# SymbioticLab/FedScale

Measured on AMD Instinct MI355X. Metric: client-updates/sec + HBM GB/s, device-resident FedAvg reduce of KxP fp32, higher is better.
Workload: dtype f32

## Files before the change

### fedscale_amd/csrc/clip_reduce.hip

```cpp
#pragma clang fp contract(off)

#include <hip/hip_runtime.h>
#include <stdint.h>

#include "../../include/fedclip.h"
#include "fa_device.h"
#include "fa_common.h"

namespace {

struct NormGeo {
  int V, U, waves, grid_pct;
};
constexpr NormGeo NQ_NARROW{8, 4, 2, 400};
constexpr NormGeo NQ_WIDE{16, 2, 4, 75};
constexpr int64_t NQ_WIDE_MIN_P = 4LL << 20;
constexpr NormGeo norm_geo(int64_t P) { return P >= NQ_WIDE_MIN_P ? NQ_WIDE : NQ_NARROW; }

struct NormArgs {
  const f4* x;
  int64_t ld4;
  int64_t P4f;
  int64_t tiles;
  int n;
  const f4* last;
  double* ws;
};

__device__ __forceinline__ double sq_acc(double acc, f4 t, f4 l) {
  const f4 d = t - l;
  acc = __builtin_fma((double)d.x, (double)d.x, acc);
  acc = __builtin_fma((double)d.y, (double)d.y, acc);
  acc = __builtin_fma((double)d.z, (double)d.z, acc);
  acc = __builtin_fma((double)d.w, (double)d.w, acc);
  return acc;
}

template <int NQ_V, int NQ_U, int NQ_WAVES>
__global__ __launch_bounds__(64 * NQ_WAVES) void k_row_sqnorm(NormArgs r) {
  constexpr int64_t NQ_TILE4 = 64 * NQ_V;
  const int lane = threadIdx.x & 63;
  const int wave = threadIdx.x >> 6;
  const f4 z4 = f4{0.f, 0.f, 0.f, 0.f};
  for (int64_t wt = (int64_t)blockIdx.x * NQ_WAVES + wave; wt < r.tiles; wt += (int64_t)gridDim.x * NQ_WAVES) {
    const int64_t c0 = wt * NQ_TILE4 + lane;
    bool ok[NQ_V];
    f4 l[NQ_V];
#pragma unroll
    for (int j = 0; j < NQ_V; ++j) {
      ok[j] = (c0 + 64 * j) < r.P4f;
      l[j] = ok[j] ? r.last[c0 + 64 * j] : z4;
    }
    const f4* row = r.x + c0;
    double* w = r.ws + wt;
    int k = 0;
    for (; k + NQ_U <= r.n; k += NQ_U) {
      f4 t[NQ_U][NQ_V];
#pragma unroll
      for (int u = 0; u < NQ_U; ++u)
#pragma unroll
        for (int j = 0; j < NQ_V; ++j) t[u][j] = ok[j] ? __builtin_nontemporal_load(row + u * r.ld4 + 64 * j) : z4;
#pragma unroll
      for (int u = 0; u < NQ_U; ++u) {
        double acc = 0.0;
#pragma unroll
        for (int j = 0; j < NQ_V; ++j) acc = sq_acc(acc, t[u][j], l[j]);
        acc = wave_sum(acc);
        if (lane == 0) w[(int64_t)(k + u) * r.tiles] = acc;
      }
      row += NQ_U * r.ld4;
    }
    for (; k < r.n; ++k) {
      double acc = 0.0;
#pragma unroll
      for (int j = 0; j < NQ_V; ++j)
        acc = sq_acc(acc, ok[j] ? __builtin_nontemporal_load(row + 64 * j) : z4, l[j]);
      acc = wave_sum(acc);
      if (lane == 0) w[(int64_t)k * r.tiles] = acc;
      row += r.ld4;
    }
  }
}

__global__ __launch_bounds__(64) void k_sqnorm_sum(const double* __restrict__ ws, int64_t tiles,
                                                   const float* __restrict__ x, int64_t ld, int64_t P4f, int64_t P,
                                                   const float* __restrict__ last, double* __restrict__ sq) {
  const int64_t k = blockIdx.x;
  const int lane = threadIdx.x;
  double acc = 0.0;
  for (int64_t t = lane; t < tiles; t += 64) acc = acc + ws[k * tiles + t];
  acc = wave_sum(acc);
  if (lane == 0) {
    for (int64_t p = 4 * P4f; p < P; ++p) {
      const float d = x[k * ld + p] - last[p];
      acc = __builtin_fma((double)d, (double)d, acc);
    }
    sq[k] = acc;
  }
}

int64_t norm_tiles(int64_t P) {
  const int64_t tile4 = 64 * norm_geo(P).V;
  return (P / 4 + tile4 - 1) / tile4;
}
int64_t norm_grid(int64_t cus, int64_t P) {
  const NormGeo g = norm_geo(P);
  const int64_t wgs = (norm_tiles(P) + g.waves - 1) / g.waves;
  const int64_t cap = cus * g.grid_pct / 100 > 0 ? cus * g.grid_pct / 100 : 1;
  return wgs < cap ? wgs : cap;
}

__global__ __launch_bounds__(256) void k_clip_coef(const double* __restrict__ sq, int n, double M,
                                                   float* __restrict__ c, int32_t* rejected) {
  const int i = blockIdx.x * 256 + threadIdx.x;
  if (i >= n) return;
  const double s = sq[i];
  float ck = 0.0f;
  if (!__builtin_isfinite(s)) {
    atomicAdd(rejected, 1);
  } else {
    const double rk = M / (sqrt(s) + 1e-6);
    ck = rk < 1.0 ? (float)rk : 1.0f;
  }
  c[i] = ck;
}

constexpr int FCL_WAVES = 4;

struct ClipArgs {
  const f4* x;
  int64_t ld4;
  int64_t P4;
  int64_t P;
  int64_t c0;
  int64_t ntiles;
  int n;
  int flags;
  const f4* last;
  const float* coef;
  const f4* acc_in;
  float* out;
};

template <int V, int U>
__device__ __forceinline__ void clip_tile(const ClipArgs& r, int64_t tile, int lane, int wave) {
  const int64_t c0 = r.c0 + (tile * FCL_WAVES + wave) * (64LL * V) + lane;
  const f4 z4 = f4{0.f, 0.f, 0.f, 0.f};
  bool ok[V];
  f4 l[V], s[V];
#pragma unroll
  for (int j = 0; j < V; ++j) {
    ok[j] = (c0 + 64 * j) < r.P4;
    l[j] = ok[j] ? r.last[c0 + 64 * j] : z4;
    s[j] = ((r.flags & FA_ACCUMULATE) && ok[j]) ? r.acc_in[c0 + 64 * j] : z4;
  }
  const f4* row = r.x + c0;
  int k = 0;
  for (; k + U <= r.n; k += U) {
    f4 t[U][V];
#pragma unroll
    for (int u = 0; u < U; ++u)
#pragma unroll
      for (int j = 0; j < V; ++j) t[u][j] = ok[j] ? __builtin_nontemporal_load(row + u * r.ld4 + 64 * j) : z4;
#pragma unroll
    for (int u = 0; u < U; ++u) {
      const float ck = r.coef[k + u];
      if (ck != 0.0f) {
#pragma unroll
        for (int j = 0; j < V; ++j) s[j] = s[j] + ck * (t[u][j] - l[j]);
      }
    }
    row += U * r.ld4;
  }
  for (; k < r.n; ++k) {
    const float ck = r.coef[k];
    if (ck != 0.0f) {
#pragma unroll
      for (int j = 0; j < V; ++j) {
        const f4 t = ok[j] ? __builtin_nontemporal_load(row + 64 * j) : z4;
        s[j] = s[j] + ck * (t - l[j]);
      }
    }
    row += r.ld4;
  }
#pragma unroll
  for (int j = 0; j < V; ++j) {
    if (!ok[j]) continue;
    const int64_t p = 4 * (c0 + 64 * j);
    if (p + 4 <= r.P) {
      *reinterpret_cast<f4*>(r.out + p) = s[j];
    } else {
      r.out[p] = s[j].x;
      if (p + 1 < r.P) r.out[p + 1] = s[j].y;
      if (p + 2 < r.P) r.out[p + 2] = s[j].z;
    }
  }
}

template <int V, int U, bool LOOP>
__global__ __launch_bounds__(64 * FCL_WAVES) void k_reduce_clip(ClipArgs r) {
  const int lane = threadIdx.x & 63;
  const int wave = threadIdx.x >> 6;
  if (LOOP) {
    for (int64_t tile = blockIdx.x; tile < r.ntiles; tile += gridDim.x) clip_tile<V, U>(r, tile, lane, wave);
  } else {
    clip_tile<V, U>(r, blockIdx.x, lane, wave);
  }
}

constexpr StripGeo FCL_GEO{FCL_WAVES, {16, 8, 2}, {1, 4, 8}, 75, 256};
static_assert(FCL_PLAN_FIELDS == STRIP_PLAN_FIELDS, "fcl_reduce_plan's row is strip_plan_export's");

int64_t clip_strips(int64_t P) { return ((P + 3) / 4 + 63) / 64; }

template <int V, int U>
void launch_one(ClipArgs r, const StripLaunch& l, hipStream_t st) {
  r.c0 = l.strip0 * 64;
  r.ntiles = l.tiles;
  const dim3 grid((unsigned)l.grid), blk(64 * FCL_WAVES);
  if constexpr (V == FCL_GEO.V[0]) {
    if (l.grid < l.tiles) {
      hipLaunchKernelGGL((k_reduce_clip<V, U, true>), grid, blk, 0, st, r);
      return;
    }
  }
  hipLaunchKernelGGL((k_reduce_clip<V, U, false>), grid, blk, 0, st, r);
}

void launch_level(const ClipArgs& r, const StripLaunch& l, hipStream_t st) {
  if (l.level == 0)
    launch_one<FCL_GEO.V[0], FCL_GEO.U[0]>(r, l, st);
  else if (l.level == 1)
    launch_one<FCL_GEO.V[1], FCL_GEO.U[1]>(r, l, st);
  else
    launch_one<FCL_GEO.V[2], FCL_GEO.U[2]>(r, l, st);
}

__device__ __forceinline__ float finish1(float ch, float l, float z, float sigma, float denom, bool noise,
                                         float& m) {
  m = __fdiv_rn(ch, denom);
  if (noise) m = m + sigma * z;
  return l + m;
}

__global__ __launch_bounds__(256) void k_clip_finish(const f4* __restrict__ chain, const f4* __restrict__ last,
                                                     const f4* __restrict__ z, float sigma, float denom, int64_t P,
                                                     float* out, float* mean_delta, float* mirror) {
  const bool noise = sigma > 0.0f;
  const int64_t P4 = (P + 3) / 4;
  for (int64_t c = (int64_t)blockIdx.x * 256 + threadIdx.x; c < P4; c += (int64_t)gridDim.x * 256) {
    const f4 ch = chain[c], l = last[c];
    const f4 zz = noise ? z[c] : f4{0.f, 0.f, 0.f, 0.f};
    float mm[4], oo[4];
#pragma unroll
    for (int i = 0; i < 4; ++i) oo[i] = finish1(ch[i], l[i], zz[i], sigma, denom, noise, mm[i]);
    const f4 m = f4{mm[0], mm[1], mm[2], mm[3]}, o = f4{oo[0], oo[1], oo[2], oo[3]};
    const int64_t p = 4 * c;
    if (p + 4 <= P) {
      *reinterpret_cast<f4*>(out + p) = o;
      if (mean_delta) *reinterpret_cast<f4*>(mean_delta + p) = m;
      if (mirror) *reinterpret_cast<f4*>(mirror + p) = o;
    } else {
      for (int i = 0; i < (int)(P - p); ++i) {
        out[p + i] = oo[i];
        if (mean_delta) mean_delta[p + i] = mm[i];
        if (mirror) mirror[p + i] = oo[i];
      }
    }
  }
}

}

extern "C" int32_t fcl_abi_version(void) { return FCL_ABI_VERSION; }

extern "C" int64_t fcl_workspace_bytes(int32_t n, int64_t P) {
  if (n < 0 || P < 0) return refuse(FA_E_ARG, "fcl_workspace_bytes: negative n=%d or P=%lld", n, (long long)P);
  const int64_t b = (int64_t)n * norm_tiles(P) * 8;
  return b > 8 ? b : 8;
}

extern "C" int64_t fcl_norm_plan(int32_t cus, int64_t P, int64_t* plan_out) {
  if (cus <= 0 || P < 0 || !plan_out)
    return refuse(FA_E_ARG, "fcl_norm_plan: bad arguments (cus=%d P=%lld)", cus, (long long)P);
  const int64_t tiles = norm_tiles(P);
  plan_out[0] = tiles;
  plan_out[1] = norm_grid(cus, P);
  plan_out[2] = norm_geo(P).waves;
  plan_out[3] = 256 * norm_geo(P).V;
  return tiles > 0 ? 2 : 1;
}

extern "C" int fcl_row_sqnorms(const float* x, int64_t ld, int32_t n, int64_t P, const float* last, double* sq,
                               double* workspace, int64_t workspace_bytes, fa_stream_t stream) {
  if (n <= 0) return refuse(FA_E_ARG, "fcl_row_sqnorms: n=%d rows, needs n >= 1", n);
  if (P < 0 || ld < P) return refuse(FA_E_ARG, "fcl_row_sqnorms: ld=%lld < P=%lld or negative P", (long long)ld, (long long)P);
  if (ld % 4 != 0) return refuse(FA_E_ARG, "fcl_row_sqnorms: ld=%lld must be a multiple of 4 elements", (long long)ld);
  if (!x || !last || !sq || !workspace) return refuse(FA_E_ARG, "fcl_row_sqnorms: x, last, sq or workspace is NULL");
  if (!aligned16(x) || !aligned16(last)) return refuse(FA_E_ARG, "fcl_row_sqnorms: x and last must be 16-byte aligned");
  if (((uintptr_t)sq & 7u) || ((uintptr_t)workspace & 7u))
    return refuse(FA_E_ARG, "fcl_row_sqnorms: sq and workspace must be 8-byte aligned");
  const int64_t tiles = norm_tiles(P);
  const int64_t need = fcl_workspace_bytes(n, P);
  if (workspace_bytes < need)
    return refuse(FA_E_ARG, "fcl_row_sqnorms: workspace of %lld bytes, needs %lld (fcl_workspace_bytes)",
                  (long long)workspace_bytes, (long long)need);
  const int64_t P4c = (P + 3) / 4;
  FA_DEVICE_SCOPE("fcl_row_sqnorms", stream, sq);
  FA_OPERAND("x", x, (uint64_t)((int64_t)(n - 1) * ld + P4c * 4) * 4);
  FA_OPERAND("last", last, (uint64_t)P4c * 16);
  FA_OPERAND("sq", sq, (uint64_t)n * 8);
  FA_OPERAND("workspace", workspace, (uint64_t)need);
  const int cus = cu_count();
  if (cus <= 0) return fail(FA_E_HIP, "fcl_row_sqnorms: no CU count for device %d", fa_scope_device());
  hipStream_t st = (hipStream_t)stream;
  if (tiles > 0) {
    NormArgs r{};
    r.x = reinterpret_cast<const f4*>(x); r.ld4 = ld / 4; r.P4f = P / 4; r.tiles = tiles; r.n = n;
    r.last = reinterpret_cast<const f4*>(last); r.ws = workspace;
    const dim3 grid((unsigned)norm_grid(cus, P));
    if (P >= NQ_WIDE_MIN_P)
      hipLaunchKernelGGL((k_row_sqnorm<NQ_WIDE.V, NQ_WIDE.U, NQ_WIDE.waves>), grid, dim3(64 * NQ_WIDE.waves), 0, st, r);
    else
      hipLaunchKernelGGL((k_row_sqnorm<NQ_NARROW.V, NQ_NARROW.U, NQ_NARROW.waves>), grid, dim3(64 * NQ_NARROW.waves),
                         0, st, r);
    const int e = check_launch("fcl_row_sqnorms");
    if (e) return e;
  }
  hipLaunchKernelGGL(k_sqnorm_sum, dim3((unsigned)n), dim3(64), 0, st, workspace, tiles, x, ld, P / 4, P, last, sq);
  return check_launch("fcl_row_sqnorms");
}

extern "C" int fcl_clip_coefs(const double* sq, int32_t n, double max_norm, float* c, int32_t* rejected,
                              fa_stream_t stream) {
  if (n <= 0) return refuse(FA_E_ARG, "fcl_clip_coefs: n=%d rows, needs n >= 1", n);
  if (!(max_norm > 0.0) || !__builtin_isfinite(max_norm))
    return refuse(FA_E_ARG, "fcl_clip_coefs: max_norm=%g must be finite and > 0", max_norm);
  if (!sq || !c || !rejected) return refuse(FA_E_ARG, "fcl_clip_coefs: sq, c or rejected is NULL");
  if (((uintptr_t)sq & 7u) || ((uintptr_t)c & 3u) || ((uintptr_t)rejected & 3u))
    return refuse(FA_E_ARG, "fcl_clip_coefs: sq must be 8-byte, c and rejected 4-byte aligned");
  FA_DEVICE_SCOPE("fcl_clip_coefs", stream, c);
  FA_OPERAND("sq", sq, (uint64_t)n * 8);
  FA_OPERAND("c", c, (uint64_t)n * 4);
  FA_OPERAND("rejected", rejected, 4);
  hipLaunchKernelGGL(k_clip_coef, dim3((unsigned)((n + 255) / 256)), dim3(256), 0, (hipStream_t)stream, sq, n,
                     max_norm, c, rejected);
  return check_launch("fcl_clip_coefs");
}

extern "C" int64_t fcl_reduce_plan(int32_t cus, int32_t K, int64_t P, int64_t* plan_out, int32_t cap) {
  if (cus <= 0 || K < 0 || P < 0 || cap < 0 || (cap > 0 && !plan_out))
    return refuse(FA_E_ARG, "fcl_reduce_plan: bad arguments (cus=%d K=%d P=%lld cap=%d)", cus, K, (long long)P, cap);
  return strip_plan_export(cus, clip_strips(P), FCL_GEO, plan_out, cap);
}

extern "C" int fcl_reduce(const float* x, int64_t ld, int32_t n, int64_t P, const float* last, const float* c,
                          const float* acc_in, float* out, int32_t flags, fa_stream_t stream) {
  if (flags & ~FA_ACCUMULATE) return refuse(FA_E_ARG, "fcl_reduce: unknown flags %d (0 or FA_ACCUMULATE)", flags);
  if (n < 0 || P < 0 || ld < P) return refuse(FA_E_ARG, "fcl_reduce: ld=%lld < P=%lld, or negative n=%d / P", (long long)ld, (long long)P, n);
  if (ld % 4 != 0) return refuse(FA_E_ARG, "fcl_reduce: ld=%lld must be a multiple of 4 elements", (long long)ld);
  if ((flags & FA_ACCUMULATE) && !acc_in) return refuse(FA_E_ARG, "fcl_reduce: FA_ACCUMULATE without acc_in");
  if (n == 0 && !(flags & FA_ACCUMULATE)) return refuse(FA_E_ARG, "fcl_reduce: n=0 rows with nothing to accumulate");
  if (n > 0 && (!x || !c)) return refuse(FA_E_ARG, "fcl_reduce: x or c is NULL");
  if (!last || !out) return refuse(FA_E_ARG, "fcl_reduce: last or out is NULL");
  if (!aligned16(x) || !aligned16(last)) return refuse(FA_E_ARG, "fcl_reduce: x and last must be 16-byte aligned");
  if (!aligned16(out) || !aligned16(acc_in)) return refuse(FA_E_ARG, "fcl_reduce: out and acc_in must be 16-byte aligned");
  if ((uintptr_t)c & 3u) return refuse(FA_E_ARG, "fcl_reduce: c must be 4-byte aligned");
  if (P == 0) return FA_OK;
  const int64_t P4 = (P + 3) / 4;
  if (P4 / (64 * FCL_WAVES) > 0x7fffffffLL) return refuse(FA_E_RANGE, "fcl_reduce: P too large");
  FA_DEVICE_SCOPE("fcl_reduce", stream, out);
  FA_OPERAND("x", x, n > 0 ? (uint64_t)((int64_t)(n - 1) * ld + P4 * 4) * 4 : 0);
  FA_OPERAND("last", last, (uint64_t)P4 * 16);
  FA_OPERAND("c", c, (uint64_t)n * 4);
  FA_OPERAND("acc_in", (flags & FA_ACCUMULATE) ? acc_in : nullptr, (uint64_t)P4 * 16);
  FA_OPERAND("out", out, (uint64_t)P * 4);
  const int cus = cu_count();
  if (cus <= 0) return fail(FA_E_HIP, "fcl_reduce launch plan: no CU count for device %d", fa_scope_device());
  ClipArgs r{};
  r.x = reinterpret_cast<const f4*>(x); r.ld4 = ld / 4; r.P4 = P4; r.P = P; r.n = n; r.flags = flags;
  r.last = reinterpret_cast<const f4*>(last); r.coef = c; r.acc_in = reinterpret_cast<const f4*>(acc_in);
  r.out = out;
  StripLaunch l[3];
  const int nl = strip_plan(cus, clip_strips(P), FCL_GEO, l);
  for (int i = 0; i < nl; ++i) {
    launch_level(r, l[i], (hipStream_t)stream);
    const int e = check_launch("fcl_reduce");
    if (e) return e;
  }
  return FA_OK;
}

extern "C" int fcl_finish(const float* chain, const float* last, const float* z, float sigma, float denom, int64_t P,
                          float* out, float* mean_delta_out, float* mirror, fa_stream_t stream) {
  if (P < 0) return refuse(FA_E_ARG, "fcl_finish: negative P=%lld", (long long)P);
  if (!(sigma >= 0.0f) || !__builtin_isfinite(sigma)) return refuse(FA_E_ARG, "fcl_finish: sigma=%g must be finite and >= 0", (double)sigma);
  if (!(denom > 0.0f)) return refuse(FA_E_ARG, "fcl_finish: denom=%g must be > 0", (double)denom);
  if (!chain || !last || !out) return refuse(FA_E_ARG, "fcl_finish: chain, last or out is NULL");
  if (sigma > 0.0f && !z) return refuse(FA_E_ARG, "fcl_finish: sigma > 0 without z");
  if (!aligned16(chain) || !aligned16(last) || !aligned16(z))
    return refuse(FA_E_ARG, "fcl_finish: chain, last and z must be 16-byte aligned");
  if (!aligned16(out) || !aligned16(mean_delta_out) || !aligned16(mirror))
    return refuse(FA_E_ARG, "fcl_finish: out, mean_delta_out and mirror must be 16-byte aligned");
  if (P == 0) return FA_OK;
  const int64_t P4 = (P + 3) / 4;
  FA_DEVICE_SCOPE("fcl_finish", stream, out);
  FA_OPERAND("chain", chain, (uint64_t)P4 * 16);
  FA_OPERAND("last", last, (uint64_t)P4 * 16);
  FA_OPERAND("z", sigma > 0.0f ? z : nullptr, (uint64_t)P4 * 16);
  FA_OPERAND("out", out, (uint64_t)P * 4);
  FA_OPERAND("mean_delta_out", mean_delta_out, (uint64_t)P * 4);
  FA_HOST_OK_OPERAND("mirror", mirror, (uint64_t)P * 4);
  const int cus = cu_count();
  if (cus <= 0) return fail(FA_E_HIP, "fcl_finish: no CU count for device %d", fa_scope_device());
  int64_t g = (P4 + 255) / 256;
  if (g > (int64_t)cus * 8) g = (int64_t)cus * 8;
  hipLaunchKernelGGL(k_clip_finish, dim3((unsigned)g), dim3(256), 0, (hipStream_t)stream,
                     reinterpret_cast<const f4*>(chain), reinterpret_cast<const f4*>(last),
                     reinterpret_cast<const f4*>(z), sigma, denom, P, out, mean_delta_out, mirror);
  return check_launch("fcl_finish");
}
```

### fedscale_amd/csrc/fa_common.h

```cpp
#pragma once

#include <hip/hip_runtime.h>
#include <stdarg.h>
#include <stdint.h>
#include <stdio.h>

#include "fa_device.h"

typedef float f4 __attribute__((ext_vector_type(4)));

__attribute__((format(printf, 2, 3))) static inline int fail(int code, const char* fmt, ...) {
  char buf[512];
  va_list ap;
  va_start(ap, fmt);
  vsnprintf(buf, sizeof(buf), fmt, ap);
  va_end(ap);
  return fa_internal_set_error(code, buf);
}
__attribute__((format(printf, 2, 3))) static inline int refuse(int code, const char* fmt, ...) {
  char msg[400], buf[512];
  va_list ap;
  va_start(ap, fmt);
  vsnprintf(msg, sizeof(msg), fmt, ap);
  va_end(ap);
  snprintf(buf, sizeof(buf), "%s (nothing was launched)", msg);
  return fa_internal_set_error(code, buf);
}
static inline int check_launch(const char* what) {
  hipError_t e = hipGetLastError();
  if (e != hipSuccess) return fail(FA_E_HIP, "%s: launch failed: %s", what, hipGetErrorString(e));
  return FA_OK;
}
static inline bool aligned16(const void* p) { return ((uintptr_t)p & 15u) == 0; }

static inline int cu_count() {
  static int cache[64];
  const int dev = fa_scope_device();
  if (dev < 0 || dev >= 64) return 0;
  if (cache[dev] > 0) return cache[dev];
  int cus = 0;
  if (hipDeviceGetAttribute(&cus, hipDeviceAttributeMultiprocessorCount, dev) != hipSuccess) {
    (void)hipGetLastError();
    return 0;
  }
  cache[dev] = cus;
  return cus;
}

__device__ __forceinline__ double wave_sum(double v) {
#pragma unroll
  for (int m = 32; m >= 1; m >>= 1) v = v + __shfl_xor(v, m, 64);
  return v;
}

struct StripGeo {
  int waves;
  int V[3], U[3];
  int cap_pct;
  int strip_cols;
};
struct StripLaunch {
  int level;
  int64_t strip0, tiles, grid;
};

static inline int strip_plan(int64_t cus, int64_t strips, const StripGeo& g, StripLaunch out[3]) {
  if (strips <= 0 || cus <= 0) return 0;
  const int64_t S = strips;
  const int64_t cap = cus * g.cap_pct / 100 > 0 ? cus * g.cap_pct / 100 : 1;
  const int64_t span0 = (int64_t)g.waves * g.V[0], span1 = (int64_t)g.waves * g.V[1],
                span2 = (int64_t)g.waves * g.V[2];
  const int64_t t0 = (S + span0 - 1) / span0;
  if (t0 * 100 >= cap * 85) {
    const int64_t rounds = (t0 + cap - 1) / cap;
    out[0] = StripLaunch{0, 0, t0, (t0 + rounds - 1) / rounds};
    return 1;
  }
  int n = 0;
  int64_t s = 0;
  const int64_t n1 = S / span1;
  if (n1 > 0 && 2 * n1 >= cus) {
    out[n++] = StripLaunch{1, 0, n1, n1};
    s = n1 * span1;
  }
  if (s < S) {
    const int64_t t2 = (S - s + span2 - 1) / span2;
    out[n++] = StripLaunch{2, s, t2, t2};
  }
  return n;
}

constexpr int STRIP_PLAN_FIELDS = 6;
static inline int strip_plan_export(int64_t cus, int64_t strips, const StripGeo& g, int64_t* plan_out, int cap) {
  StripLaunch l[3];
  const int n = strip_plan(cus, strips, g, l);
  for (int i = 0; i < n && i < cap; ++i) {
    int64_t* o = plan_out + (int64_t)STRIP_PLAN_FIELDS * i;
    o[0] = g.V[l[i].level];
    o[1] = g.U[l[i].level];
    o[2] = l[i].strip0 * g.strip_cols;
    o[3] = l[i].tiles;
    o[4] = g.V[l[i].level];
    o[5] = l[i].grid;
  }
  return n;
}
```

### fedscale_amd/csrc/fedagg.hip

```cpp
#pragma clang fp contract(off)

#include <hip/hip_runtime.h>
#include <stdint.h>
#include <stdarg.h>
#include <stdio.h>
#include <stdlib.h>
#include <string.h>

#include <unistd.h>

#include <atomic>
#include <condition_variable>
#include <functional>
#include <mutex>
#include <thread>
#include <vector>

#include "../../include/fedagg.h"
#include "fa_device.h"
#include "fa_common.h"

#define FA_ABI_VERSION 5

#ifndef FA_BUILD_ID
#define FA_BUILD_ID "unset"
#endif
#ifndef FA_BUILD_DEFS
#define FA_BUILD_DEFS ""
#endif
__attribute__((used)) static const char fa_build_marker[] = "FA_BUILD_ID=" FA_BUILD_ID;

#ifndef FA_TUNING
#define FA_TUNING 0
#endif

static thread_local char g_err[512] = "";

static uint64_t rows_bytes(int64_t K, int64_t ld, int64_t P, int elem = 4) {
  return K > 0 ? (uint64_t)((K - 1) * ld + (P + 3) / 4 * 4) * elem : 0;
}
static uint64_t cols_bytes(int64_t P) { return (uint64_t)((P + 3) / 4) * 16; }

extern "C" __attribute__((visibility("hidden"))) int fa_internal_set_error(int code, const char* msg) {
  snprintf(g_err, sizeof(g_err), "%s", msg);
  return code;
}

static std::atomic<int64_t> g_unranged{0};
static std::atomic<int> g_strict_operands{0};
extern "C" __attribute__((visibility("hidden"))) void fa_internal_note_unranged(void) {
  g_unranged.fetch_add(1, std::memory_order_relaxed);
}
extern "C" __attribute__((visibility("hidden"))) int fa_internal_strict_operands(void) {
  return g_strict_operands.load(std::memory_order_relaxed);
}
extern "C" int64_t fa_unranged_operands(void) { return g_unranged.load(std::memory_order_relaxed); }
extern "C" int fa_set_strict_operands(int32_t on) { return g_strict_operands.exchange(on ? 1 : 0); }

extern "C" int fa_abi_version(void) { return FA_ABI_VERSION; }
extern "C" const char* fa_build_id(void) { return fa_build_marker + sizeof("FA_BUILD_ID=") - 1; }
extern "C" const char* fa_build_defs(void) { return FA_BUILD_DEFS; }
extern "C" int fa_pointer_kind(const void* p) { return fa_host_mapped(p); }
extern "C" const char* fa_last_error_string(void) { return g_err; }

#ifndef FA_RED_NT
#define FA_RED_NT 1
#endif
__device__ __forceinline__ f4 ldnt(const f4* p) {
#if FA_RED_NT
  return __builtin_nontemporal_load(p);
#else
  return *p;
#endif
}

#ifndef FA_RED_BUF
#define FA_RED_BUF 0
#endif
#if !FA_TUNING && (FA_RED_BUF || !FA_RED_NT)
#error "FA_RED_BUF / FA_RED_NT=0 are tuning knobs: build with -DFA_TUNING=1"
#endif
#ifndef FA_RED_AUX
#define FA_RED_AUX 2
#endif
__device__ __forceinline__ f4 ldrow(const f4* ub, int lane, int j) {
#if FA_RED_BUF
  const __amdgpu_buffer_rsrc_t rs = __builtin_amdgcn_make_buffer_rsrc(const_cast<f4*>(ub), (short)0, 0x7fffffff,
                                                                     0x00020000);
  return __builtin_bit_cast(f4, __builtin_amdgcn_raw_buffer_load_b128(rs, (lane + 64 * j) * 16, 0, FA_RED_AUX));
#else
  return ldnt(ub + lane + 64 * j);
#endif
}

__device__ __forceinline__ float sgnf(float x) {
  return x > 0.f ? 1.f : (x < 0.f ? -1.f : x);
}
__device__ __forceinline__ double sgnd(double x) { return x > 0.0 ? 1.0 : (x < 0.0 ? -1.0 : x); }

__device__ __forceinline__ int64_t f32_to_i64(float v) {
  return (v > -9223372036854775808.f && v < 9223372036854775808.f) ? (int64_t)v : INT64_MIN;
}

__device__ __forceinline__ float yogi_elem(float cur, float last, float& m, float& v, float eta, float tau,
                                           float beta, float omb, float omb2) {
  const float g = cur - last;
  const float g2 = g * g;
  m = beta * m + omb * g;
  v = v - (omb2 * g2) * sgnf(v - g2);
  const float den = __builtin_sqrtf(v) + tau;
  const float lr = __frcp_rn(den) * eta;
  return last + lr * m;
}

__device__ __forceinline__ f4 yogi4(f4 cur, f4 last, f4& M, f4& V, float eta, float tau, float beta, float omb,
                                    float omb2) {
  float m[4] = {M.x, M.y, M.z, M.w}, v[4] = {V.x, V.y, V.z, V.w};
  float c[4] = {cur.x, cur.y, cur.z, cur.w}, l[4] = {last.x, last.y, last.z, last.w}, o[4];
#pragma unroll
  for (int i = 0; i < 4; ++i) o[i] = yogi_elem(c[i], l[i], m[i], v[i], eta, tau, beta, omb, omb2);
  M = f4{m[0], m[1], m[2], m[3]};
  V = f4{v[0], v[1], v[2], v[3]};
  return f4{o[0], o[1], o[2], o[3]};
}

enum { EPI_CHAIN = 0, EPI_MEAN = 1, EPI_YOGI = 2 };

struct RedArgs {
  const float* x;
  int64_t ld4;
  int64_t P4;
  int64_t col0;
  int64_t ntiles;
  int sw;
  int K;
  int flags;
  const float* a;
  const float* acc_in;
  float* out;
  float denom;
  const float* last;
  float* m;
  float* v;
  float* mean_out;
  float eta, tau, beta, omb, omb2;
};

#ifndef FA_XCD_REMAP
#define FA_XCD_REMAP 0
#endif
#ifndef FA_RED_WAVES
#define FA_RED_WAVES 4
#endif
#ifndef FA_PIPE
#define FA_PIPE 0
#endif
#if !FA_TUNING && (FA_XCD_REMAP || FA_PIPE || FA_RED_WAVES != 4)
#error "FA_XCD_REMAP / FA_PIPE / FA_RED_WAVES are tuning knobs: build with -DFA_TUNING=1"
#endif
template <int V, int U, int EPI, bool W, bool FULL, bool PIPE = false>
__device__ __forceinline__ void reduce_tile(const RedArgs& r, int64_t tile, int lane, int wave) {
  const f4* __restrict__ xp = reinterpret_cast<const f4*>(r.x);
  const int sw = FULL ? V : r.sw;
  const int64_t c0 = r.col0 + (tile * FA_RED_WAVES + wave) * (64LL * sw) + lane;
#if FA_RED_BUF
  const f4* xu = xp + (int64_t)__builtin_amdgcn_readfirstlane((int)(c0 - lane));
#else
  const f4* xu = xp + (c0 - lane);
#endif

  bool ok[V];
#pragma unroll
  for (int j = 0; j < V; ++j) ok[j] = (FULL || j < sw) && (c0 + 64 * j) < r.P4;

  f4 s[V];
  int k = 0;
  if (r.flags & FA_ACCUMULATE) {
    const f4* ain = reinterpret_cast<const f4*>(r.acc_in);
#pragma unroll
    for (int j = 0; j < V; ++j) s[j] = ok[j] ? ain[c0 + 64 * j] : f4{0.f, 0.f, 0.f, 0.f};
  } else {
    const float w0 = W ? r.a[0] : 1.f;
#pragma unroll
    for (int j = 0; j < V; ++j) {
      f4 t = ok[j] ? ldrow(xu, lane, j) : f4{0.f, 0.f, 0.f, 0.f};
      s[j] = W ? t * w0 : t;
    }
    k = 1;
  }

  const f4* row = xu + (int64_t)k * r.ld4;
  auto load_group = [&](f4(&t)[U][V], const f4* rw) {
#pragma unroll
    for (int u = 0; u < U; ++u)
#pragma unroll
      for (int j = 0; j < V; ++j)
        t[u][j] = ok[j] ? ldrow(rw + u * r.ld4, lane, j) : f4{0.f, 0.f, 0.f, 0.f};
  };
  auto add_group = [&](const f4(&t)[U][V], int k0) {
#pragma unroll
    for (int u = 0; u < U; ++u) {
      const float w = W ? r.a[k0 + u] : 1.f;
#pragma unroll
      for (int j = 0; j < V; ++j) s[j] = W ? s[j] + w * t[u][j] : s[j] + t[u][j];
    }
  };
  if ((PIPE || FA_PIPE) && k + U <= r.K) {
    f4 ta[U][V], tb[U][V];
    load_group(ta, row);
    row += U * r.ld4;
    for (;;) {
      const bool more = k + 2 * U <= r.K;
      if (more) load_group(tb, row), row += U * r.ld4;
      add_group(ta, k);
      k += U;
      if (!more) break;
      const bool more2 = k + 2 * U <= r.K;
      if (more2) load_group(ta, row), row += U * r.ld4;
      add_group(tb, k);
      k += U;
      if (!more2) break;
    }
  }
  for (; k + U <= r.K; k += U) {
    f4 t[U][V];
    load_group(t, row);
    add_group(t, k);
    row += U * r.ld4;
  }
  for (; k < r.K; ++k) {
    const float w = W ? r.a[k] : 1.f;
#pragma unroll
    for (int j = 0; j < V; ++j) {
      f4 t = ok[j] ? ldrow(row, lane, j) : f4{0.f, 0.f, 0.f, 0.f};
      s[j] = W ? s[j] + w * t : s[j] + t;
    }
    row += r.ld4;
  }

#pragma unroll
  for (int j = 0; j < V; ++j) {
    if (!ok[j]) continue;
    const int64_t c = c0 + 64 * j;
    if (EPI == EPI_CHAIN) {
      reinterpret_cast<f4*>(r.out)[c] = s[j];
    } else if (EPI == EPI_MEAN) {
      f4 o;
      o.x = __fdiv_rn(s[j].x, r.denom);
      o.y = __fdiv_rn(s[j].y, r.denom);
      o.z = __fdiv_rn(s[j].z, r.denom);
      o.w = __fdiv_rn(s[j].w, r.denom);
      reinterpret_cast<f4*>(r.out)[c] = o;
      if (r.mean_out) reinterpret_cast<f4*>(r.mean_out)[c] = o;
    } else {
      const f4 L = reinterpret_cast<const f4*>(r.last)[c];
      f4 M, Vv;
      if (r.flags & FA_YOGI_INIT) {
        M = f4{0.f, 0.f, 0.f, 0.f};
        Vv = f4{r.tau, r.tau, r.tau, r.tau};
      } else {
        M = reinterpret_cast<const f4*>(r.m)[c];
        Vv = reinterpret_cast<const f4*>(r.v)[c];
      }
      const f4 cur = f4{__fdiv_rn(s[j].x, r.denom), __fdiv_rn(s[j].y, r.denom), __fdiv_rn(s[j].z, r.denom),
                        __fdiv_rn(s[j].w, r.denom)};
      const f4 o = yogi4(cur, L, M, Vv, r.eta, r.tau, r.beta, r.omb, r.omb2);
      if (r.mean_out) reinterpret_cast<f4*>(r.mean_out)[c] = cur;
      reinterpret_cast<f4*>(r.m)[c] = M;
      reinterpret_cast<f4*>(r.v)[c] = Vv;
      reinterpret_cast<f4*>(r.out)[c] = o;
    }
  }
}

template <int V, int U, int EPI, bool W, bool LOOP, bool FULL = true, bool PIPE = false>
__global__ __launch_bounds__(64 * FA_RED_WAVES) void k_reduce(RedArgs r) {
  const int lane = threadIdx.x & 63;
  const int wave = threadIdx.x >> 6;
  if (LOOP) {
    int64_t b = blockIdx.x;
#if FA_XCD_REMAP
    {
      const int64_t G = gridDim.x, q = G / 8, rem = G % 8, x = b % 8;
      b = x * q + (x < rem ? x : rem) + b / 8;
    }
#endif
    for (int64_t tile = b; tile < r.ntiles; tile += gridDim.x) reduce_tile<V, U, EPI, W, FULL, PIPE>(r, tile, lane, wave);
  } else {
    reduce_tile<V, U, EPI, W, FULL, PIPE>(r, blockIdx.x, lane, wave);
  }
}

#if defined(FA_RED_V) && !FA_TUNING
#error "FA_RED_V (a single fixed variant) is a tuning build: add -DFA_TUNING=1"
#endif
#ifdef FA_RED_V
#define FA_LEVELS 1
#define FA_L0_V FA_RED_V
#define FA_L0_U FA_RED_U
#else
#define FA_LEVELS 4
#define FA_L0_V 32
#define FA_L0_U 1
#define FA_L1_V 16
#define FA_L1_U 4
#define FA_L2_V 8
#define FA_L2_U 4
#define FA_L3_V 2
#define FA_L3_U 8
#endif
#ifndef FA_GRID_CAP_PCT
#define FA_GRID_CAP_PCT 75
#endif

static thread_local int64_t* g_plan_count = nullptr;
#define FA_RED_LAUNCH(kern, grid, block, st, args)         \
  do {                                                     \
    if (g_plan_count)                                      \
      ++*g_plan_count;                                     \
    else                                                   \
      hipLaunchKernelGGL(kern, grid, block, 0, st, args);  \
  } while (0)

#if FA_TUNING
template <int V, int U, int EPI, bool W>
static int resident_blocks() {
  static int cache[64];
  const int dev = fa_scope_device();
  if (dev < 0 || dev >= 64) return 0;
  if (cache[dev] > 0) return cache[dev];
  int per_cu = 0;
  if (hipOccupancyMaxActiveBlocksPerMultiprocessor(
          &per_cu, reinterpret_cast<const void*>(&k_reduce<V, U, EPI, W, false>), 64 * FA_RED_WAVES, 0) != hipSuccess)
    return 0;
  cache[dev] = per_cu * cu_count();
  return cache[dev];
}

template <int V, int U, int EPI, bool W>
static int64_t launch_level(RedArgs r, int64_t col, int64_t col_end, bool full_waves_only, int64_t cap,
                            hipStream_t st) {
  const int64_t span = 64LL * FA_RED_WAVES * V;
  r.sw = V;
  int64_t nblk = (col_end - col + span - 1) / span;
  if (full_waves_only) {
    const int64_t R = resident_blocks<V, U, EPI, W>();
    if (R <= 0) return col;
    const int64_t total = nblk;
    nblk = ((col_end - col) / span) / R * R;
    if (total - nblk >= (R * 9) / 10) nblk = total;
  }
  if (nblk <= 0) return col;
  r.col0 = col;
  r.ntiles = nblk;
  if (cap > 0 && nblk > cap) {
    const int64_t rounds = (nblk + cap - 1) / cap;
    const int64_t grid = (nblk + rounds - 1) / rounds;
    FA_RED_LAUNCH((k_reduce<V, U, EPI, W, true>), dim3((unsigned)grid), dim3(64 * FA_RED_WAVES), st, r);
  } else {
    FA_RED_LAUNCH((k_reduce<V, U, EPI, W, false>), dim3((unsigned)nblk), dim3(64 * FA_RED_WAVES), st, r);
  }
  const int64_t end = col + nblk * span;
  return (full_waves_only && end < col_end) ? end : col_end;
}
#endif

#ifndef FA_BAL_GRID
#define FA_BAL_GRID 224
#endif
#ifndef FA_BAL_MIN_SW
#define FA_BAL_MIN_SW 5
#endif
#ifndef FA_BAL_MIN_WORK
#define FA_BAL_MIN_WORK 1000
#endif
#ifndef FA_BAL_SHORT_K
#define FA_BAL_SHORT_K 200
#endif
#ifndef FA_CAP_SW_MAX
#define FA_CAP_SW_MAX 32
#endif
static_assert(FA_CAP_SW_MAX >= 8 && FA_CAP_SW_MAX <= 32, "FA_CAP_SW_MAX: 8..32");
#ifndef FA_WINDOWS
#define FA_WINDOWS 1
#endif
template <int V, int U, int EPI, bool W>
static void launch_balanced(RedArgs r, int64_t sw, int64_t rounds, hipStream_t st) {
  const int64_t S = (r.P4 + 63) / 64;
  r.col0 = 0;
  r.sw = (int)sw;
  r.ntiles = (S + (int64_t)FA_RED_WAVES * sw - 1) / ((int64_t)FA_RED_WAVES * sw);
  const int64_t grid = (r.ntiles + rounds - 1) / rounds;
  const dim3 blk(64 * FA_RED_WAVES);
#if FA_TUNING || !FA_WINDOWS || FA_CAP_SW_MAX != 32
  if (grid < r.ntiles) {
    if (sw == V)
      FA_RED_LAUNCH((k_reduce<V, U, EPI, W, true, true>), dim3((unsigned)grid), blk, st, r);
    else
      FA_RED_LAUNCH((k_reduce<V, U, EPI, W, true, false>), dim3((unsigned)grid), blk, st, r);
    return;
  }
#endif
  (void)grid;
  if (sw == V) {
    FA_RED_LAUNCH((k_reduce<V, U, EPI, W, false, true>), dim3((unsigned)r.ntiles), blk, st, r);
  } else {
    FA_RED_LAUNCH((k_reduce<V, U, EPI, W, false, false>), dim3((unsigned)r.ntiles), blk, st, r);
  }
}

#ifndef FA_WIN_FULL_MIN
#define FA_WIN_FULL_MIN 33
#endif
template <int EPI, bool W>
static void launch_window(RedArgs r, int64_t s0, int64_t ns, int64_t cap, hipStream_t st) {
  int64_t sw = (ns + (int64_t)FA_RED_WAVES * cap - 1) / ((int64_t)FA_RED_WAVES * cap);
  if (sw >= FA_WIN_FULL_MIN && sw < 32) sw = 32;
  r.col0 = s0 * 64;
  r.P4 = (s0 + ns) * 64 < r.P4 ? (s0 + ns) * 64 : r.P4;
  r.sw = (int)sw;
  r.ntiles = (ns + (int64_t)FA_RED_WAVES * sw - 1) / ((int64_t)FA_RED_WAVES * sw);
  const dim3 grid((unsigned)r.ntiles), blk(64 * FA_RED_WAVES);
  if (sw == 32)
    FA_RED_LAUNCH((k_reduce<32, 1, EPI, W, false, true>), grid, blk, st, r);
  else if (sw > 16)
    FA_RED_LAUNCH((k_reduce<32, 1, EPI, W, false, false>), grid, blk, st, r);
  else if (sw == 16)
    FA_RED_LAUNCH((k_reduce<16, 2, EPI, W, false, true>), grid, blk, st, r);
  else
    FA_RED_LAUNCH((k_reduce<16, 2, EPI, W, false, false>), grid, blk, st, r);
}

#ifndef FA_SHORT_PIPE
#define FA_SHORT_PIPE 1
#endif
template <int EPI, bool W>
static void launch_short(RedArgs r, hipStream_t st) {
  const int64_t span = 64LL * FA_RED_WAVES * 4;
  r.col0 = 0;
  r.sw = 4;
  r.ntiles = (r.P4 + span - 1) / span;
  FA_RED_LAUNCH((k_reduce<4, 4, EPI, W, false, true, true>), dim3((unsigned)r.ntiles), dim3(64 * FA_RED_WAVES), st, r);
}
template <int EPI, bool W>
static int launch_plan(const RedArgs& r, hipStream_t st) {
#if FA_LEVELS == 1
#if defined(FA_RED_GRID) && FA_RED_GRID > 0
  launch_level<FA_L0_V, FA_L0_U, EPI, W>(r, 0, r.P4, false, FA_RED_GRID, st);
#else
  launch_level<FA_L0_V, FA_L0_U, EPI, W>(r, 0, r.P4, false, 0, st);
#endif
  return FA_OK;
#else
  const int64_t cus = cu_count();
  if (cus <= 0) return fail(FA_E_HIP, "k_reduce launch plan: no CU count for device %d", fa_scope_device());
  const int64_t cap = cus * FA_GRID_CAP_PCT / 100;
#if FA_BAL_GRID > 0
  {
    const int64_t S = (r.P4 + 63) / 64;
    const int64_t g1 = r.K < FA_BAL_SHORT_K ? cus : cap;
    const int64_t sw1 = (S + (int64_t)FA_RED_WAVES * g1 - 1) / ((int64_t)FA_RED_WAVES * g1);
    if (sw1 > 32) {
      const int64_t per_round = (int64_t)FA_RED_WAVES * FA_CAP_SW_MAX * cap;
      const int64_t R = (S + per_round - 1) / per_round;
      if (FA_WINDOWS && FA_CAP_SW_MAX == 32) {
        const int64_t Sw = (S + R - 1) / R;
        for (int64_t s0 = 0; s0 < S; s0 += Sw) launch_window<EPI, W>(r, s0, S - s0 < Sw ? S - s0 : Sw, cap, st);
        return FA_OK;
      }
      const int64_t sw = (S + (int64_t)FA_RED_WAVES * R * cap - 1) / ((int64_t)FA_RED_WAVES * R * cap);
      if (sw > 16)
        launch_balanced<32, 1, EPI, W>(r, sw, R, st);
      else
        launch_balanced<16, 2, EPI, W>(r, sw, R, st);
      return FA_OK;
    }
    if (sw1 >= 8) {
      if (sw1 > 16)
        launch_balanced<32, 1, EPI, W>(r, sw1, 1, st);
      else
        launch_balanced<16, 2, EPI, W>(r, sw1, 1, st);
      return FA_OK;
    }
    const int64_t gb = cus * FA_BAL_GRID / 256;
    const int64_t swb = (S + (int64_t)FA_RED_WAVES * gb - 1) / ((int64_t)FA_RED_WAVES * gb);
    if (swb >= FA_BAL_MIN_SW && (int64_t)r.K * swb >= FA_BAL_MIN_WORK) {
      if (swb > 8)
        launch_balanced<16, 2, EPI, W>(r, swb, 1, st);
      else
        launch_balanced<8, 4, EPI, W>(r, swb, 1, st);
      return FA_OK;
    }
  }
#endif
#if FA_SHORT_PIPE
  launch_short<EPI, W>(r, st);
  return FA_OK;
#elif FA_TUNING
  const int64_t span0 = 64LL * FA_RED_WAVES * FA_L0_V;
  const int64_t tiles0 = (r.P4 + span0 - 1) / span0;
  if (tiles0 * 20 >= cap * 17) {
    launch_level<FA_L0_V, FA_L0_U, EPI, W>(r, 0, r.P4, false, cap, st);
    return FA_OK;
  }
  int64_t col = launch_level<FA_L0_V, FA_L0_U, EPI, W>(r, 0, r.P4, true, 0, st);
  if (col < r.P4) col = launch_level<FA_L1_V, FA_L1_U, EPI, W>(r, col, r.P4, true, 0, st);
  if (col < r.P4) col = launch_level<FA_L2_V, FA_L2_U, EPI, W>(r, col, r.P4, true, 0, st);
  if (col < r.P4) launch_level<FA_L3_V, FA_L3_U, EPI, W>(r, col, r.P4, false, 0, st);
  return FA_OK;
#else
#error "FA_SHORT_PIPE=0 / FA_BAL_GRID=0 fall back to the level cascade: a tuning build (-DFA_TUNING=1)"
#endif
#endif
}

template <int EPI>
static int launch_reduce(const RedArgs& r, hipStream_t st, const char* what) {
  if (r.P4 <= 0) return FA_OK;
  if (r.P4 / (64 * FA_RED_WAVES) > 0x7fffffffLL) return fail(FA_E_RANGE, "%s: P too large", what);
  const int e = r.a ? launch_plan<EPI, true>(r, st) : launch_plan<EPI, false>(r, st);
  if (e) return e;
  return check_launch(what);
}

extern "C" int64_t fa_reduce_launches(int32_t K, int64_t P, int32_t weighted) {
  if (K <= 0 || P <= 0) return 0;
  RedArgs r{};
  r.P4 = (P + 3) / 4;
  r.K = K;
  int64_t n = 0;
  g_plan_count = &n;
  const int e = weighted ? launch_plan<EPI_MEAN, true>(r, nullptr) : launch_plan<EPI_MEAN, false>(r, nullptr);
  g_plan_count = nullptr;
  return e ? e : n;
}

static int check_reduce_args(const char* what, const float* x, int64_t ld, int32_t K, int64_t P,
                             const float* acc_in, const float* out, int32_t flags) {
  if (K < 0 || P < 0 || ld < P) return fail(FA_E_ARG, "%s: bad sizes (ld < P or negative)", what);
  if (ld % 4 != 0) return fail(FA_E_ARG, "%s: ld=%lld must be a multiple of 4", what, (long long)ld);
  if ((flags & FA_ACCUMULATE) && !acc_in) return fail(FA_E_ARG, "%s: FA_ACCUMULATE without acc_in", what);
  if (K == 0 && !(flags & FA_ACCUMULATE)) return fail(FA_E_ARG, "%s: K == 0 with nothing to accumulate", what);
  if (K > 0 && !x) return fail(FA_E_ARG, "%s: x is NULL", what);
  if (!out) return fail(FA_E_ARG, "%s: out is NULL", what);
  if (!aligned16(x) || !aligned16(out) || !aligned16(acc_in))
    return fail(FA_E_ARG, "%s: device pointers must be 16-byte aligned", what);
  return FA_OK;
}

extern "C" int fa_reduce(const float* x, int64_t ld, int32_t K, int64_t P, const float* a, const float* acc_in,
                         float* out, float denom, int32_t flags, fa_stream_t stream) {
  int e = check_reduce_args("fa_reduce", x, ld, K, P, acc_in, out, flags);
  if (e) return e;
  if (P == 0) return FA_OK;
  RedArgs r{};
  r.x = x; r.ld4 = ld / 4; r.P4 = (P + 3) / 4; r.K = K; r.flags = flags; r.a = a; r.acc_in = acc_in;
  r.out = out; r.denom = denom;
  FA_DEVICE_SCOPE("fa_reduce", stream, out);
  FA_HOST_OK_OPERAND("x", x, rows_bytes(K, ld, P));
  FA_OPERAND("a", a, (uint64_t)K * 4);
  FA_OPERAND("acc_in", (flags & FA_ACCUMULATE) ? acc_in : nullptr, cols_bytes(P));
  FA_OPERAND("out", out, cols_bytes(P));
  hipStream_t st = (hipStream_t)stream;
  if (flags & FA_FINALIZE) return launch_reduce<EPI_MEAN>(r, st, "fa_reduce");
  return launch_reduce<EPI_CHAIN>(r, st, "fa_reduce");
}

extern "C" int fa_reduce_parts(int32_t n, const float* const* x, const int64_t* ld, const int32_t* K,
                               const int64_t* P, const float* const* acc_in, float* const* out, float denom,
                               const int32_t* flags, void* const* streams) {
  if (n < 1 || !x || !ld || !K || !P || !acc_in || !out || !flags || !streams)
    return fail(FA_E_ARG, "fa_reduce_parts: NULL table or n < 1");
  char what[48];
  for (int i = 0; i < n; ++i) {
    snprintf(what, sizeof(what), "fa_reduce_parts[%d]", i);
    int e = check_reduce_args(what, x[i], ld[i], K[i], P[i], acc_in[i], out[i], flags[i]);
    if (e) return e;
    if (!streams[i]) return fail(FA_E_ARG, "%s: NULL stream (one stream per part's GPU)", what);
    if (P[i] == 0) continue;
// ... 1596 lines not shown
```

Before: 71730.

## Add software-pipelined unpredicated row walker for interior tiles in reduce kernels

Adds a RowWalk template that double-buffers row loads: it issues the next half-group of nontemporal loads while consuming the previous one, with sched_barrier pins to hold that order. Fully in-bounds (interior) tiles in the FedAvg reduce, clip reduce and row-sqnorm kernels now take this path without per-lane bound predicates, and read per-row coefficients through scalar constant-address loads. It also adds min-waves launch bounds sized from register use. The aim is more memory-level parallelism and fewer predicate and VALU instructions in the HBM-bound loop, at the cost of more register pressure and code size.

```diff
diff --git a/fedscale_amd/csrc/clip_reduce.hip b/fedscale_amd/csrc/clip_reduce.hip
--- a/fedscale_amd/csrc/clip_reduce.hip
+++ b/fedscale_amd/csrc/clip_reduce.hip
@@ -36,8 +36,29 @@
   return acc;
 }
 
+template <int V>
+struct SqRows {
+  static constexpr bool HEADED = false;
+  const f4 (&l)[V];
+  double* w;
+  int64_t tiles;
+  int lane;
+  double acc;
+  static __device__ __forceinline__ f4 ld(const f4* p, int lane) { return __builtin_nontemporal_load(p + lane); }
+  template <int J0, int J1, bool HEAD>
+  __device__ __forceinline__ void rows(int k, const f4* v) {
+    if (J0 == 0) acc = 0.0;
+#pragma unroll
+    for (int j = J0; j < J1; ++j) acc = sq_acc(acc, v[j - J0], l[j]);
+    if (J1 == V) {
+      acc = wave_sum(acc);
+      if (lane == 0) w[(int64_t)k * tiles] = acc;
+    }
+  }
+};
+
 template <int NQ_V, int NQ_U, int NQ_WAVES>
-__global__ __launch_bounds__(64 * NQ_WAVES) void k_row_sqnorm(NormArgs r) {
+__global__ __launch_bounds__(64 * NQ_WAVES, 2) void k_row_sqnorm(NormArgs r) {
   constexpr int64_t NQ_TILE4 = 64 * NQ_V;
   const int lane = threadIdx.x & 63;
   const int wave = threadIdx.x >> 6;
@@ -51,9 +72,19 @@
       ok[j] = (c0 + 64 * j) < r.P4f;
       l[j] = ok[j] ? r.last[c0 + 64 * j] : z4;
     }
-    const f4* row = r.x + c0;
     double* w = r.ws + wt;
     int k = 0;
+#if !FA_ROW_PRED
+    if constexpr (NQ_V <= 8) {
+      const int64_t cw = (int64_t)__builtin_amdgcn_readfirstlane((int)wt) * NQ_TILE4;
+      if (cw + NQ_TILE4 <= r.P4f) {
+        SqRows<NQ_V> f{l, w, r.tiles, lane, 0.0};
+        RowWalk<NQ_V, NQ_U, f4, decltype(f)>(r.x + cw, lane, r.ld4, f).walk(0, r.n);
+        k = r.n;
+      }
+    }
+#endif
+    const f4* row = r.x + c0 + (int64_t)k * r.ld4;
     for (; k + NQ_U <= r.n; k += NQ_U) {
       f4 t[NQ_U][NQ_V];
 #pragma unroll
@@ -142,6 +173,23 @@
   float* out;
 };
 
+template <int V>
+struct ClipRows {
+  static constexpr bool HEADED = false;
+  f4 (&s)[V];
+  const f4 (&l)[V];
+  const float* coef;
+  static __device__ __forceinline__ f4 ld(const f4* p, int lane) { return __builtin_nontemporal_load(p + lane); }
+  template <int J0, int J1, bool HEAD>
+  __device__ __forceinline__ void rows(int k, const f4* v) {
+    const float ck = ld_row_scalar(coef, k);
+    if (ck != 0.0f) {
+#pragma unroll
+      for (int j = J0; j < J1; ++j) s[j] = s[j] + ck * (v[j - J0] - l[j]);
+    }
+  }
+};
+
 template <int V, int U>
 __device__ __forceinline__ void clip_tile(const ClipArgs& r, int64_t tile, int lane, int wave) {
   const int64_t c0 = r.c0 + (tile * FCL_WAVES + wave) * (64LL * V) + lane;
@@ -154,8 +202,18 @@
     l[j] = ok[j] ? r.last[c0 + 64 * j] : z4;
     s[j] = ((r.flags & FA_ACCUMULATE) && ok[j]) ? r.acc_in[c0 + 64 * j] : z4;
   }
-  const f4* row = r.x + c0;
   int k = 0;
+#if !FA_ROW_PRED
+  if constexpr (V != 8) {
+    const int64_t cw = r.c0 + (tile * FCL_WAVES + __builtin_amdgcn_readfirstlane(wave)) * (64LL * V);
+    if (cw + 64 * V <= r.P4) {
+      ClipRows<V> f{s, l, r.coef};
+      RowWalk<V, U, f4, decltype(f)>(r.x + cw, lane, r.ld4, f).walk(0, r.n);
+      k = r.n;
+    }
+  }
+#endif
+  const f4* row = r.x + c0 + (int64_t)k * r.ld4;
   for (; k + U <= r.n; k += U) {
     f4 t[U][V];
 #pragma unroll
@@ -183,10 +241,12 @@
     }
     row += r.ld4;
   }
+  int64_t ce = c0;
+  asm volatile("" : "+v"(ce));
 #pragma unroll
   for (int j = 0; j < V; ++j) {
     if (!ok[j]) continue;
-    const int64_t p = 4 * (c0 + 64 * j);
+    const int64_t p = 4 * (ce + 64 * j);
     if (p + 4 <= r.P) {
       *reinterpret_cast<f4*>(r.out + p) = s[j];
     } else {
@@ -197,8 +257,9 @@
   }
 }
 
+constexpr int clip_min_waves(int V, int U) { return 8 * V + 4 * U * V <= 80 ? 4 : 8 * V + 4 * U * V <= 192 ? 2 : 1; }
 template <int V, int U, bool LOOP>
-__global__ __launch_bounds__(64 * FCL_WAVES) void k_reduce_clip(ClipArgs r) {
+__global__ __launch_bounds__(64 * FCL_WAVES, clip_min_waves(V, U)) void k_reduce_clip(ClipArgs r) {
   const int lane = threadIdx.x & 63;
   const int wave = threadIdx.x >> 6;
   if (LOOP) {
diff --git a/fedscale_amd/csrc/fa_common.h b/fedscale_amd/csrc/fa_common.h
--- a/fedscale_amd/csrc/fa_common.h
+++ b/fedscale_amd/csrc/fa_common.h
@@ -52,6 +52,128 @@
   for (int m = 32; m >= 1; m >>= 1) v = v + __shfl_xor(v, m, 64);
   return v;
 }
+
+#ifndef FA_ROW_PRED
+#define FA_ROW_PRED 0
+#endif
+#if FA_ROW_PRED && !(defined(FA_TUNING) && FA_TUNING)
+#error "FA_ROW_PRED (predicated row loads on every tile) is a tuning knob: build with -DFA_TUNING=1"
+#endif
+
+__device__ __forceinline__ float ld_row_scalar(const float* p, int k) {
+  typedef const float __attribute__((address_space(4))) * cptr;
+  return ((cptr)(uintptr_t)p)[k];
+}
+
+template <int V, int U, typename T, typename F>
+struct RowWalk {
+  static_assert(U == 1 || U == 2 || U == 4 || U == 8, "halves are whole rows; remainder dispatch");
+  static_assert(U > 1 || V % 2 == 0, "halves are whole strips");
+  static constexpr int HU = U / 2;
+  static constexpr int HV = V / 2;
+  T t[U][V];
+  const T* row;
+  int lane;
+  int64_t ld;
+  F& f;
+
+  __device__ __forceinline__ RowWalk(const T* row_, int lane_, int64_t ld_, F& f_)
+      : row(row_), lane(lane_), ld(ld_), f(f_) {}
+
+  static __device__ __forceinline__ void pin() { __builtin_amdgcn_sched_barrier(0); }
+
+  template <int U0, int U1, int J0 = 0, int J1 = V>
+  __device__ __forceinline__ void issue() {
+#pragma unroll
+    for (int u = U0; u < U1; ++u)
+#pragma unroll
+      for (int j = J0; j < J1; ++j) t[u][j] = F::ld(row + u * ld + 64 * j, lane);
+    pin();
+  }
+  template <int U0, int U1, bool FIRST>
+  __device__ __forceinline__ void use(int k) {
+    if constexpr (U0 < U1) {
+      f.template rows<0, V, (FIRST && U0 == 0)>(k + U0, t[U0]);
+      use<U0 + 1, U1, FIRST>(k);
+    } else {
+      pin();
+    }
+  }
+  template <int J, int J1, bool FIRST>
+  __device__ __forceinline__ void use_strips(int k) {
+    if constexpr (J < J1) {
+      f.template rows<J, J + 1, FIRST>(k, &t[0][J]);
+      pin();
+      use_strips<J + 1, J1, FIRST>(k);
+    }
+  }
+
+  template <int R, bool FIRST>
+  __device__ __forceinline__ void part(int k) {
+    issue<0, R>();
+    use<0, R, FIRST>(k);
+  }
+  template <bool FIRST>
+  __device__ __forceinline__ void tail(int k, int rem) {
+    if constexpr (U >= 2) {
+      if (rem == 1) part<1, FIRST>(k);
+    }
+    if constexpr (U >= 4) {
+      if (rem == 2) part<2, FIRST>(k);
+      if (rem == 3) part<3, FIRST>(k);
+    }
+    if constexpr (U >= 8) {
+      if (rem == 4) part<4, FIRST>(k);
+      if (rem == 5) part<5, FIRST>(k);
+      if (rem == 6) part<6, FIRST>(k);
+      if (rem == 7) part<7, FIRST>(k);
+    }
+  }
+
+  template <bool FIRST, bool MORE>
+  __device__ __forceinline__ void turn(int k) {
+    if constexpr (U == 1) {
+      issue<0, 1, HV, V>();
+      use_strips<0, HV, FIRST>(k);
+      row += ld;
+      if (MORE) issue<0, 1, 0, HV>();
+      use_strips<HV, V, FIRST>(k);
+    } else {
+      issue<HU, U>();
+      use<0, HU, FIRST>(k);
+      row += U * ld;
+      if (MORE) issue<0, HU>();
+      use<HU, U, false>(k);
+    }
+  }
+
+  __device__ __forceinline__ void walk(int k, int K) {
+    if (k >= K) return;
+    int nfull = (K - k) / U;
+    const int rem = (K - k) % U;
+    if (nfull == 0) {
+      tail<F::HEADED>(k, rem);
+      return;
+    }
+    if constexpr (U == 1) issue<0, 1, 0, HV>(); else issue<0, HU>();
+    if constexpr (F::HEADED) {
+      if (nfull > 1) {
+        turn<true, true>(k);
+        k += U;
+        --nfull;
+        for (; nfull > 1; --nfull, k += U) turn<false, true>(k);
+        turn<false, false>(k);
+      } else {
+        turn<true, false>(k);
+      }
+    } else {
+      for (; nfull > 1; --nfull, k += U) turn<false, true>(k);
+      turn<false, false>(k);
+    }
+    k += U;
+    tail<false>(k, rem);
+  }
+};
 
 struct StripGeo {
   int waves;
diff --git a/fedscale_amd/csrc/fedagg.hip b/fedscale_amd/csrc/fedagg.hip
--- a/fedscale_amd/csrc/fedagg.hip
+++ b/fedscale_amd/csrc/fedagg.hip
@@ -158,6 +158,67 @@
 #if !FA_TUNING && (FA_XCD_REMAP || FA_PIPE || FA_RED_WAVES != 4)
 #error "FA_XCD_REMAP / FA_PIPE / FA_RED_WAVES are tuning knobs: build with -DFA_TUNING=1"
 #endif
+#ifndef FA_RED_RING32
+#define FA_RED_RING32 0
+#endif
+#ifndef FA_RED_RING8
+#define FA_RED_RING8 0
+#endif
+#if !FA_TUNING && (FA_RED_RING32 || FA_RED_RING8)
+#error "FA_RED_RING32 / FA_RED_RING8 are tuning knobs: build with -DFA_TUNING=1"
+#endif
+constexpr bool red_has_interior(int V, int U) {
+  return V == 16 && U == 2 ? false
+         : V == 32         ? FA_RED_RING32 != 0
+         : V == 8          ? FA_RED_RING8 != 0
+                           : U == 2 || U == 4 || U == 8;
+}
+template <int V, bool W, bool INIT0>
+struct RedRows {
+  static constexpr bool HEADED = INIT0;
+  f4 (&s)[V];
+  const float* a;
+  bool init0;
+  static __device__ __forceinline__ f4 ld(const f4* p, int lane) { return ldnt(p + lane); }
+  template <int J0, int J1, bool HEAD>
+  __device__ __forceinline__ void rows(int k, const f4* v) {
+    const float w = W ? ld_row_scalar(a, k) : 1.f;
+    if (INIT0 && HEAD && init0) {
+#pragma unroll
+      for (int j = J0; j < J1; ++j) s[j] = W ? v[j - J0] * w : v[j - J0];
+    } else {
+#pragma unroll
+      for (int j = J0; j < J1; ++j) s[j] = W ? s[j] + w * v[j - J0] : s[j] + v[j - J0];
+    }
+  }
+};
+template <int V, int U, bool W, bool PIPE>
+__device__ __forceinline__ void reduce_interior(const RedArgs& r, int64_t tile, int lane, int wave, f4 (&s)[V]) {
+  const int64_t cw = r.col0 + (tile * FA_RED_WAVES + __builtin_amdgcn_readfirstlane(wave)) * (64LL * V);
+  const int64_t c0 = cw + lane;
+  const f4* row = reinterpret_cast<const f4*>(r.x) + cw;
+  const bool acc = (r.flags & FA_ACCUMULATE) != 0;
+  int k = 0;
+  if (acc) {
+    const f4* ain = reinterpret_cast<const f4*>(r.acc_in);
+#pragma unroll
+    for (int j = 0; j < V; ++j) s[j] = ain[c0 + 64 * j];
+  } else if (!PIPE) {
+    const float w0 = W ? r.a[0] : 1.f;
+#pragma unroll
+    for (int j = 0; j < V; ++j) {
+      const f4 t = ldnt(row + 64 * j + lane);
+      s[j] = W ? t * w0 : t;
+    }
+    k = 1;
+  } else {
+#pragma unroll
+    for (int j = 0; j < V; ++j) s[j] = f4{0.f, 0.f, 0.f, 0.f};
+  }
+  RedRows<V, W, PIPE> f{s, r.a, !acc};
+  RowWalk<V, U, f4, decltype(f)>(row + k * r.ld4, lane, r.ld4, f).walk(k, r.K);
+}
+
 template <int V, int U, int EPI, bool W, bool FULL, bool PIPE = false>
 __device__ __forceinline__ void reduce_tile(const RedArgs& r, int64_t tile, int lane, int wave) {
   const f4* __restrict__ xp = reinterpret_cast<const f4*>(r.x);
@@ -175,6 +236,13 @@
 
   f4 s[V];
   int k = 0;
+  bool interior = false;
+#if !FA_ROW_PRED && !FA_RED_BUF
+  if constexpr (FULL && red_has_interior(V, U)) interior = __builtin_amdgcn_readfirstlane((int)((c0 - lane) + 64LL * V <= r.P4)) != 0;
+#endif
+  if (interior) {
+    if constexpr (FULL && red_has_interior(V, U)) reduce_interior<V, U, W, PIPE>(r, tile, lane, wave, s);
+  } else {
   if (r.flags & FA_ACCUMULATE) {
     const f4* ain = reinterpret_cast<const f4*>(r.acc_in);
 #pragma unroll
@@ -236,6 +304,7 @@
       s[j] = W ? s[j] + w * t : s[j] + t;
     }
     row += r.ld4;
+  }
   }
 
 #pragma unroll
@@ -273,8 +342,11 @@
   }
 }
 
+constexpr int red_min_waves(int V, int U, bool PIPE) {
+  return FA_RED_WAVES != 4 ? 1 : PIPE ? 3 : 4 * V * (U + 1) <= 192 ? 2 : 1;
+}
 template <int V, int U, int EPI, bool W, bool LOOP, bool FULL = true, bool PIPE = false>
-__global__ __launch_bounds__(64 * FA_RED_WAVES) void k_reduce(RedArgs r) {
+__global__ __launch_bounds__(64 * FA_RED_WAVES, red_min_waves(V, U, PIPE)) void k_reduce(RedArgs r) {
   const int lane = threadIdx.x & 63;
   const int wave = threadIdx.x >> 6;
   if (LOOP) {
```

Result: no change. 71630 (-0.1%).
